# Wu0409/DuPL

Measured on AMD Instinct MI355X. Metric: training img/s at 448^2, VOC dual-student ViT-B/16, phase B step, higher is better.
Workload: dtype f32 storage / accumulation / results; Linear GEMMs (forward, dgrad, wgrad), attention (forward, backward) and the decoder convs as fp32-equivalent f16x3 split products on the f16 MFMA (operands as fp16 hi / lo planes, 3 products per block, fp32 accumulate; error vs fp64 <= the f32 MFMA kernels'); CA

## Files before the change

dupl_amd/csrc/gemm_split.hip:

```cpp
#include "split_frag.h"
#include "../../include/dupl_hip.h"

#ifndef G16_ABL
#define G16_ABL 0
#endif

namespace {

constexpr int TBK = 32;

template <bool F1>
__global__ __launch_bounds__(256) void split_kernel(const float* __restrict__ x, __half* __restrict__ hi, __half* __restrict__ lo,
                                                    long n4, float scale) {
    for (long i = (long)blockIdx.x * blockDim.x + threadIdx.x; i < n4; i += (long)gridDim.x * blockDim.x) {
        const float4 v = reinterpret_cast<const float4*>(x)[i];
        __half h[4], l[4];
        if constexpr (F1) {
            split_f32_u(v.x * scale, h[0], l[0]);
            split_f32_u(v.y * scale, h[1], l[1]);
            split_f32_u(v.z * scale, h[2], l[2]);
            split_f32_u(v.w * scale, h[3], l[3]);
        } else {
            split_f32(v.x, h[0], l[0]);
            split_f32(v.y, h[1], l[1]);
// ... 375 lines not shown
    const bool pre_ld = !ACC && E.vec && nv == 4 && ((p.res != nullptr) != want_aux);
    const float* pre_src = want_aux ? p.aux : p.res;
    const int pre_ldm = want_aux ? p.ldaux : p.ldr;
#pragma unroll
    for (int i = 0; i < WM; ++i)
#pragma unroll
        for (int g = 0; g < 4; ++g) {
            f32x4 pq[2] = {f32x4{0.f, 0.f, 0.f, 0.f}, f32x4{0.f, 0.f, 0.f, 0.f}};
            if (pre_ld) {
#pragma unroll
                for (int k = 0; k < 2; ++k) {
                    const int row = mw + i * 32 + 8 * g + rl + 4 * k;
                    if (row < p.M) pq[k] = *reinterpret_cast<const f32x4*>(pre_src + (size_t)row * pre_ldm + col);
                }
            }
#pragma unroll
            for (int j = 0; j < WN; ++j)
#pragma unroll
                for (int q = 0; q < 4; ++q)
                {
                    float v;
                    if constexpr (SINGLE) v = accM[i][j][4 * g + q] * alpha;
                    else v = (accM[i][j][4 * g + q] + accX[SINGLE ? 0 : i][SINGLE ? 0 : j][4 * g + q] * LO_INV) * alpha;
                    side[(q + 4 * hf) * 64 + j * 32 + l31] = v;
                }
            if constexpr (ACC) {
                if (OVERW && (p.flags & DUPL_GEMM_C_FRESH)) {
                    if (nw + lane < p.N) {
#pragma unroll
                        for (int r = 0; r < 8; ++r) {
                            const int row = mw + i * 32 + 8 * g + r;
                            if (row < p.M) p.C[(size_t)row * p.ldc + nw + lane] = 0.f + side[r * 64 + lane];
                        }
                    }
                } else if (nw + lane < p.N) {
#pragma unroll
                    for (int r = 0; r < 8; ++r) {
                        const int row = mw + i * 32 + 8 * g + r;
                        if (row < p.M) {
                            float* cp = p.C + (size_t)row * p.ldc + nw + lane;
                            if constexpr (ATOM) unsafeAtomicAdd(cp, side[r * 64 + lane]);
                            else *cp += side[r * 64 + lane];
                        }
                    }
                }
            } else {
#pragma unroll
                for (int k = 0; k < 2; ++k) {
                    const int r = rl + 4 * k;
                    const f32x4 t = *reinterpret_cast<const f32x4*>(side + r * 64 + cl);
                    const int row = mw + i * 32 + 8 * g + r;
                    if (nv > 0 && row < p.M)
                        epi16_quad(p, E, row, col, nv, t, bv, amx, pq[k], pre_ld ? (want_aux ? 2 : 1) : 0);
                }
            }
        }
}

template <int WM, int WN, int NWM, int NWN>
struct RingGeom {
    static constexpr int BM = 32 * WM * NWM, BN = 32 * WN * NWN, NW = NWM * NWN;
    static constexpr int PA = BM / 16, PB = BN / 16;
    static constexpr int NP = 2 * PA + 2 * PB;
    static constexpr int STAGE = NP * 1024;
    static constexpr int PPW = NP / NW;
    static constexpr int NMF = 3 * WM * WN, NR = 2 * (WM + WN);
    static_assert(NP % NW == 0, "pieces must divide over the waves");
};

template <int BM, int BN>
struct TileOrder {
    int nbm, g_gm, nblk, q8, r8, gspan;
    __device__ __forceinline__ TileOrder(const int nbm_, const int nbn, const int g_gm_)
        : nbm(nbm_), g_gm(g_gm_), nblk(nbm_ * nbn), q8(nblk >> 3), r8(nblk & 7), gspan(g_gm_ * nbn) {}
    __device__ __forceinline__ void lid_origin(const int lid, int& m0, int& n0) const {
        const int gid = lid / gspan, gin = lid - gid * gspan;
        const int gfirst = gid * g_gm;
        const int gsz = min(nbm - gfirst, g_gm);
        m0 = (gfirst + gin % gsz) * BM;
        n0 = (gin / gsz) * BN;
    }
    __device__ __forceinline__ void tile_origin(const int bid, int& m0, int& n0) const {
        const int xcd = bid & 7, idx = bid >> 3;
        lid_origin((xcd < r8 ? xcd * (q8 + 1) : r8 * (q8 + 1) + (xcd - r8) * q8) + idx, m0, n0);
    }
    __device__ __forceinline__ bool has_tile(const int bid) const { return (bid >> 3) < q8 + ((bid & 7) < r8 ? 1 : 0); }
};

__device__ __forceinline__ void g16_dma_piece(const char*& gp, char* dst) {
    if (!(G16_ABL & 1))
        __builtin_amdgcn_global_load_lds((const __attribute__((address_space(1))) void*)gp, (__attribute__((address_space(3))) void*)dst,
                                         16, 0, 0);
    gp += TBK * 2;
}

template <int WM, int WN, int PA, int PB>
struct Frag32 {
    int a_row, b_row;
    __device__ __forceinline__ void read_frags(const char* st, const int cs, h8 (&fa)[2 * WM], h8 (&fb)[2 * WN]) const {
#pragma unroll
        for (int i = 0; i < WM; ++i) {
            fa[i] = *reinterpret_cast<const h8*>(st + a_row + i * 2048 + cs);
            fa[WM + i] = *reinterpret_cast<const h8*>(st + PA * 1024 + a_row + i * 2048 + cs);
        }
#pragma unroll
        for (int j = 0; j < WN; ++j) {
// ... 944 lines not shown
        for (; t < nt; ++t) {
            const int nb = rb + 1 == STAGES ? 0 : rb + 1;
            const char* st = smem + rb * STAGE;
            const unsigned so = (unsigned)(rb * STAGE), son = (unsigned)(nb * STAGE);
            __builtin_amdgcn_s_waitcnt(LGKM0);
            phase(std::integral_constant<int, NRI>{}, f0a, f0b, [&](auto sc) __attribute__((always_inline)) { read_r(sc, KS1, st, so, f1a, f1b); });
            if (t + 1 < nt) {
                __builtin_amdgcn_s_waitcnt(WAIT_LGKM0_VM(0));
                __builtin_amdgcn_s_barrier();
                asm volatile("" ::: "memory");
                phase(std::integral_constant<int, NRI>{}, f1a, f1b, [&](auto sc) __attribute__((always_inline)) { read_r(sc, KS0, smem + nb * STAGE, son, f0a, f0b); });
            } else {
                __builtin_amdgcn_s_waitcnt(LGKM0);
                phase(std::integral_constant<int, 0>{}, f1a, f1b, [](auto) {});
            }
            rb = nb;
        }
        asm volatile("s_waitcnt lgkmcnt(0)" ::: "memory");
        __builtin_amdgcn_s_barrier();
        asm volatile("" ::: "memory");
        const int mw = m0 + wm * (32 * WM), nw = n0 + wn * (32 * WN);
        bool more;
        if constexpr (SK) {
            pos += nt;
            more = pos < pend;
            if (more) {
                nt = min(pend - pos, ntf);
                order.lid_origin(pos / ntf, m0, n0);
                plan(m0, n0, 0);
            }
        } else if constexpr (ONESHOT) {
            more = false;
        } else {
            bid += grid;
            more = order.has_tile(bid);
            if (more) {
                order.tile_origin(bid, m0, n0);
                plan(m0, n0, 0);
            }
        }
        if (more) {
#pragma unroll
            for (int s = 0; s < STAGES; ++s) issue(s);
        }
        gemm16_epilogue_side<WM, WN, ACC != 0, true, ACC == 1, ONESHOT>(p, acc, accX_unused, reinterpret_cast<float*>(smem + STAGES * STAGE) + wave * 512,
                                                               mw, nw, lane, amx);
        if (!more) break;
    }
    if (p.amax_out)
        gemm16_amax_flush(static_cast<unsigned int*>(p.amax_out), amx, reinterpret_cast<float*>(smem + STAGES * STAGE), wave, lane,
                          NWM * NWN);
}

template <int WM, int WN, int NWM, int NWN, int WPS, bool SK, int ACC, bool AKM, bool BKM, int STAGES = 3>
__global__ __launch_bounds__(64 * NWM * NWN, WPS) void gemm_f16x3_km_kernel(const dupl_gemm16_desc p, const int g_gm) {
    gemm_f16x3_km_body<WM, WN, NWM, NWN, WPS, SK, ACC, AKM, BKM, STAGES>(p, g_gm, blockIdx.x, gridDim.x);
}

struct g16_group_args {
    dupl_gemm16_desc d[DUPL_GEMM16_GROUP_MAX];
    int first[DUPL_GEMM16_GROUP_MAX + 1];
    int n;
};
template <int WM, int WN, int NWM, int NWN, int WPS>
__global__ __launch_bounds__(64 * NWM * NWN, WPS) void gemm_f16x3_km_group_kernel(const g16_group_args g, const int g_gm) {
    const int T = g.first[g.n];
    const int xcd = blockIdx.x & 7, idx = blockIdx.x >> 3;
    const int lo = (int)((long)T * xcd / 8), hi = (int)((long)T * (xcd + 1) / 8);
    if (idx >= hi - lo) return;
    const int t = lo + idx;
    int i = 0;
#pragma unroll 1
    while (i + 1 < g.n && t >= g.first[i + 1]) ++i;
    i = __builtin_amdgcn_readfirstlane(i);
    gemm_f16x3_km_body<WM, WN, NWM, NWN, WPS, false, 2, true, true, 3, true>(g.d[i], g_gm, t - g.first[i], 1 << 28);
}

}

constexpr int G16_GROUP_M = 8;
constexpr int G16_GROUP_RING = 2;
constexpr int G16_F1_BIG_FROM = 96;

extern "C" int dupl_split_f16x2(const float* x, void* hi, void* lo, int64_t n, dupl_stream_t stream) {
    if (!x || !hi || !lo || n <= 0 || (n & 3) || (reinterpret_cast<uintptr_t>(x) & 15) || (reinterpret_cast<uintptr_t>(hi) & 7) ||
        (reinterpret_cast<uintptr_t>(lo) & 7))
        return DUPL_ERR_ARG;
    const long n4 = n / 4;
    long g = (n4 + 255) / 256;
    if (g > 8192) g = 8192;
    DUPL_LAUNCH(split_kernel<false>, dim3((unsigned)g), dim3(256), 0, (hipStream_t)stream, x, (__half*)hi, (__half*)lo, n4, 1.f);
    return dupl_launch_status();
}

extern "C" int dupl_split_f16x2b(const float* x, void* hi, void* lo, int64_t n, int32_t scale_exp, dupl_stream_t stream) {
    if (!x || !hi || !lo || n <= 0 || (n & 3) || (reinterpret_cast<uintptr_t>(x) & 15) || (reinterpret_cast<uintptr_t>(hi) & 7) ||
        (reinterpret_cast<uintptr_t>(lo) & 7) || scale_exp < 0 || scale_exp > 15)
        return DUPL_ERR_ARG;
    const long n4 = n / 4;
    long g = (n4 + 255) / 256;
    if (g > 8192) g = 8192;
    DUPL_LAUNCH(split_kernel<true>, dim3((unsigned)g), dim3(256), 0, (hipStream_t)stream, x, (__half*)hi, (__half*)lo, n4,
                       ldexpf(1.f, scale_exp));
    return dupl_launch_status();
}

static bool g16_operands_ok(const dupl_gemm16_desc& d) {
    if (d.struct_size != sizeof(dupl_gemm16_desc)) return false;
    if (!d.A_hi || !d.A_lo || !d.B_hi || !d.B_lo || d.M <= 0 || d.N <= 0 || d.K <= 0) return false;
    if ((d.K % TBK) || (d.lda % 8) || (d.ldb % 8)) return false;
    auto al16 = [](const void* q) { return (reinterpret_cast<uintptr_t>(q) & 15) == 0; };
    if (!al16(d.A_hi) || !al16(d.A_lo) || !al16(d.B_hi) || !al16(d.B_lo)) return false;
    if (d.group < 0 || d.group > 4096) return false;
    if (d.a_layout < 0 || d.a_layout > 1 || d.b_layout < 0 || d.b_layout > 1 || d.ka_valid < 0 || d.kb_valid < 0) return false;
    if (d.a_layout || d.b_layout) {
        if (d.fmt != 1 || d.K / TBK < 3) return false;
        if ((d.a_layout && (d.M & 7)) || (d.b_layout && (d.N & 7))) return false;
        if (d.ka_valid > d.K || d.kb_valid > d.K) return false;
        if ((!d.a_layout && d.ka_valid) || (!d.b_layout && d.kb_valid)) return false;
    }
    return true;
}

extern "C" int dupl_gemm_f16x3_group(const dupl_gemm16_desc* descs, int32_t n, dupl_stream_t stream) {
    if (!descs || n < 1 || n > DUPL_GEMM16_GROUP_MAX) return DUPL_ERR_ARG;
    g16_group_args g;
    g.n = n;
    int total = 0, group = 0;
    for (int i = 0; i < n; ++i) {
        const dupl_gemm16_desc& d = descs[i];
        if (!g16_operands_ok(d)) return DUPL_ERR_ARG;
        if ((d.flags & ~DUPL_GEMM_C_FRESH) != DUPL_GEMM_ACCUM || d.a_layout != 1 || d.b_layout != 1) return DUPL_ERR_ARG;
        if (!d.C || d.C_hi || d.C_lo || d.bias || d.res || d.c_rows || d.amax_out) return DUPL_ERR_ARG;
        g.d[i] = d;
        g.first[i] = total;
        const int nblk = ((d.M + 255) / 256) * ((d.N + 127) / 128);
        total += nblk;
        if (d.group) group = d.group;
    }
    g.first[n] = total;
    DUPL_LAUNCH((gemm_f16x3_km_group_kernel<2, 2, 4, 2, 2>), dim3((unsigned)(8 * ((total + 7) / 8))), dim3(512), 0, (hipStream_t)stream, g,
                       group ? group : G16_GROUP_RING);
    return dupl_launch_status();
}

static bool g16_split_rows(const dupl_gemm16_desc& d, const int M1, dupl_gemm16_desc& d1, dupl_gemm16_desc& d2) {
    d1 = d; d2 = d;
    d1.M = M1;
    d2.M = d.M - M1;
    auto adv = [&](const void* q, size_t elems, size_t bytes) { return q ? static_cast<const void*>(static_cast<const char*>(q) + elems * bytes) : nullptr; };
    d2.A_hi = adv(d.A_hi, (size_t)M1 * d.lda, 2); d2.A_lo = adv(d.A_lo, (size_t)M1 * d.lda, 2);
    d2.C = (float*)adv(d.C, (size_t)M1 * d.ldc, 4);
    d2.C_hi = (void*)adv(d.C_hi, (size_t)M1 * d.ldo, 2); d2.C_lo = (void*)adv(d.C_lo, (size_t)M1 * d.ldo, 2);
    d2.res = (const float*)adv(d.res, (size_t)M1 * d.ldr, 4);
    d2.aux = (float*)adv(d.aux, (size_t)M1 * d.ldaux, 4);
    if (d.c_rows > 0) {
        if (d.c_rows <= M1) {
            d2.c_rows = 0; d2.C = nullptr; d2.aux = nullptr; d2.flags &= ~DUPL_GEMM_STORE_PRE;
        } else { d1.c_rows = 0; d2.c_rows = d.c_rows - M1; }
    }
    return d2.C || d2.C_hi;
}

constexpr int G16_TILES[] = {
    0,
    3,
    5,
    6,
    7,
    8,
    10,
    11,
    12,
    14,
    18,
    22,
};

static int g16_tile16(const dupl_gemm16_desc& d) {
    return ((d.M + 255) / 256) * ((d.N + 255) / 256) >= G16_F1_BIG_FROM ? 18 : 22;
}
using g16_kernel_t = void (*)(dupl_gemm16_desc, int);
static void g16_launch16(const dupl_gemm16_desc& d, const int t, const bool automatic, const int group, hipStream_t s, g16_kernel_t big,
                         g16_kernel_t small) {
    auto launch = [&](g16_kernel_t k, const dupl_gemm16_desc& q, const int bn) {
        DUPL_LAUNCH(k, dim3((unsigned)(((q.M + 255) / 256) * ((q.N + bn - 1) / bn))), dim3(512), 0, s, q, group);
    };
    if (t == 22) return launch(small, d, 128);
    const int cn = (d.N + 255) / 256, rm = (d.M + 255) / 256, cus = 256;
    const int nb22 = rm * cn, full = nb22 / cus, tail = nb22 - full * cus;
    const int r_big = full > 0 ? (full * cus) / cn : 0;
    dupl_gemm16_desc d1, d2;
    if (automatic && full > 0 && tail > 0 && tail * 10 < cus * 3 && r_big > 0 && r_big < rm && !d.amax_out && g16_split_rows(d, r_big * 256, d1, d2)) {
        launch(big, d1, 256);
        launch(small, d2, 128);
    } else launch(big, d, 256);
}

static int g16_launch_hi(const dupl_gemm16_desc& d, const int tile, const int group, hipStream_t s);

extern "C" int dupl_gemm_f16x3(const dupl_gemm16_desc* d, dupl_stream_t stream) {
    if (!d) return DUPL_ERR_ARG;
    dupl_gemm16_desc hi1;
    const bool single = d->struct_size == sizeof(dupl_gemm16_desc) && d->products == 1;
    if (single) {
        hi1 = *d;
        if (!hi1.A_lo) hi1.A_lo = hi1.A_hi;
        if (!hi1.B_lo) hi1.B_lo = hi1.B_hi;
        d = &hi1;
    }
    if (!g16_operands_ok(*d)) return DUPL_ERR_ARG;
    if (d->products != 0 && d->products != 1 && d->products != 3) return DUPL_ERR_ARG;
    if (d->concurrency < 0 || d->concurrency > 8 || d->persist_blocks < 0 || d->persist_blocks > 1024 || (d->persist_blocks & 7))
        return DUPL_ERR_ARG;
    bool known_tile = false;
    for (const int t : G16_TILES) known_tile |= d->tile == t;
    if (!known_tile) return DUPL_ERR_ARG;
    const int g16_tile = d->tile, g16_concurrency = d->concurrency > 0 ? d->concurrency : 1;
    const int g16_persist_blocks = d->persist_blocks ? d->persist_blocks : (g16_concurrency >= 2 ? 192 : 256);
    const int g16_group_m = d->group ? d->group : G16_GROUP_M, g16_group_ring = d->group ? d->group : G16_GROUP_RING;
    if (!d->C && !d->C_hi) return DUPL_ERR_ARG;
    if ((d->C_hi == nullptr) != (d->C_lo == nullptr)) return DUPL_ERR_ARG;
    if ((d->flags & (DUPL_GEMM_STORE_PRE | DUPL_GEMM_MUL_DGELU | DUPL_GEMM_MUL_RELUMASK)) && !d->aux) return DUPL_ERR_ARG;
    if (d->flags & ~(DUPL_GEMM_GELU | DUPL_GEMM_RELU | DUPL_GEMM_STORE_PRE | DUPL_GEMM_ACCUM | DUPL_GEMM_MUL_DGELU |
                     DUPL_GEMM_MUL_RELUMASK))
        return DUPL_ERR_ARG;
    const bool accum = d->flags & DUPL_GEMM_ACCUM;
    if (accum && (!d->C || d->C_hi || d->bias || d->res || d->c_rows)) return DUPL_ERR_ARG;
    if (d->c_rows < 0 || (d->c_rows && (d->flags & (DUPL_GEMM_MUL_DGELU | DUPL_GEMM_MUL_RELUMASK)))) return DUPL_ERR_ARG;
    if (d->amax_out && (accum || d->c_rows || (reinterpret_cast<uintptr_t>(d->amax_out) & 3))) return DUPL_ERR_ARG;
    const bool kmajor = d->a_layout || d->b_layout;
    if (d->fmt < 0 || d->fmt > 1 || d->out_exp < 0 || d->out_exp > 15 || (d->out_exp && d->fmt != 1) ||
        (d->fmt == 1 && !kmajor && (accum || d->amax_out)))
        return DUPL_ERR_ARG;
    hipStream_t s = (hipStream_t)stream;
    if (single) {
        if (accum || kmajor) return DUPL_ERR_ARG;
        return g16_launch_hi(*d, g16_tile, g16_group_ring, s);
    }
    int ksplit = 1;
    if (accum) {
        const long tiles = (long)((d->M + 127) / 128) * ((d->N + 127) / 128);
        ksplit = (int)((512 + tiles - 1) / tiles);
        const int maxs = (d->K / TBK + 7) / 8;
        if (ksplit > maxs) ksplit = maxs;
        if (ksplit < 1) ksplit = 1;
        if (d->deterministic) ksplit = 1;
    }
    int tile = g16_tile;
    if (tile == 0) {
        const long b256 = (long)((d->M + 255) / 256) * ((d->N + 127) / 128);
        const long b128 = (long)((d->M + 127) / 128) * ((d->N + 127) / 128) * ksplit;
        const bool ring = b256 >= (g16_concurrency >= 2 ? 64 : 128);
        if (!accum && ring) tile = 10;
        else if (accum && ksplit > 1 && d->K / TBK >= 8 && b256 * (d->K / TBK) >= 10L * g16_persist_blocks &&
                 (g16_concurrency < 2 || b256 >= 64))
            tile = 11;
        else tile = b128 < 200 ? 3 : 5;
    }
    auto blocks = [&](int bm, int bn) { return dim3((unsigned)(((d->M + bm - 1) / bm) * ((d->N + bn - 1) / bn)), (unsigned)ksplit); };
    auto persist_grid = [&](const int nblk) {
        const int tx = (nblk + 7) / 8, bmax = g16_persist_blocks / 8;
        const int rounds = (tx + bmax - 1) / bmax;
        return dim3((unsigned)(8 * ((tx + rounds - 1) / rounds)));
    };
    if (kmajor) {
        const int nb21 = ((d->M + 255) / 256) * ((d->N + 127) / 128);
        const bool sk = accum && !d->deterministic && ksplit > 1;
        dupl_gemm16_desc dsk = *d;
        if (accum) {
            const int ntf = d->K / TBK;
            auto per = [&](int s_) { return (ntf + s_ - 1) / s_; };
            auto fits = [&](int s_) { return s_ > 0 && (long)nb21 * s_ <= g16_persist_blocks && per(s_) >= 3 && ntf - (s_ - 1) * per(s_) >= 3; };
            if (dsk.sk_slices > 0 && !fits(dsk.sk_slices)) dsk.sk_slices = 0;
            if (dsk.sk_slices == 0) {
                int S = nb21 > g16_persist_blocks ? -1 : g16_persist_blocks / nb21;
                while (S > 1 && (per(S) < 3 || ntf - (S - 1) * per(S) < 3)) --S;
                dsk.sk_slices = S;
            }
            if (dsk.sk_slices > 0 && !fits(dsk.sk_slices)) dsk.sk_slices = -1;
        }
        if (accum && !d->a_layout) {
            if (!d->b_layout || d->deterministic) return DUPL_ERR_ARG;
            DUPL_LAUNCH((gemm_f16x3_km_kernel<2, 2, 4, 2, 2, true, 1, false, true>), dim3((unsigned)g16_persist_blocks), dim3(512), 0, s, dsk, g16_group_ring);
        } else if (accum) {
            if (!(d->a_layout && d->b_layout)) return DUPL_ERR_ARG;
            if (sk) DUPL_LAUNCH((gemm_f16x3_km_kernel<2, 2, 4, 2, 2, true, 1, true, true>), dim3((unsigned)g16_persist_blocks), dim3(512), 0, s, dsk, g16_group_ring);
            else DUPL_LAUNCH((gemm_f16x3_km_kernel<2, 2, 4, 2, 2, false, 2, true, true>), persist_grid(nb21), dim3(512), 0, s, *d, g16_group_ring);
        } else {
            if (d->a_layout || !d->b_layout) return DUPL_ERR_ARG;
            DUPL_LAUNCH((gemm_f16x3_km_kernel<2, 2, 4, 2, 2, false, 0, false, true>), persist_grid(nb21), dim3(512), 0, s, *d, g16_group_ring);
        }
        return dupl_launch_status();
    }
    if (d->fmt == 1) {
        const int nb21 = ((d->M + 255) / 256) * ((d->N + 127) / 128);
        int t = (g16_tile == 8 || g16_tile == 12 || g16_tile == 14 || g16_tile == 18 || g16_tile == 22) ? g16_tile : g16_tile16(*d);
        if (d->K / TBK < 3 && t == 14) t = 12;
        if (t == 18 || t == 22)
            g16_launch16(*d, t, g16_tile == 0, g16_group_ring, s, gemm_f16x3_ring16_kernel<4, 2, 2, 4, 2, 2>, gemm_f16x3_ring16_kernel<2, 2, 4, 2, 2, 3>);
        else if (t == 8) DUPL_LAUNCH((gemm_f16x3_ring_kernel<4, 2, 2, 4, 2, 2, true>), blocks(256, 256), dim3(512), 0, s, *d, g16_group_ring);
        else if (t == 12) DUPL_LAUNCH((gemm_f16x3_ring_kernel<2, 2, 4, 2, 2, 3, true>), blocks(256, 128), dim3(512), 0, s, *d, g16_group_ring);
        else
            DUPL_LAUNCH((gemm_f16x3_pring_kernel<2, 2, 4, 2, 2, false, true, 3>), persist_grid(nb21), dim3(512), 0, s, *d, g16_group_ring);
        return dupl_launch_status();
    }
    if (tile == 10 && (accum || d->K / TBK < 3)) tile = 6;
    if (tile == 11 && (!accum || d->deterministic || d->K / TBK < 8)) tile = accum ? 5 : 6;
    if (tile == 11) {
        DUPL_LAUNCH((gemm_f16x3_pring_kernel<2, 2, 4, 2, 2, true>), dim3((unsigned)g16_persist_blocks), dim3(512), 0, s, *d,
                           g16_group_ring);
        return dupl_launch_status();
    }
    if (tile == 10) {
        DUPL_LAUNCH((gemm_f16x3_pring_kernel<2, 2, 4, 2, 2>), persist_grid(((d->M + 255) / 256) * ((d->N + 127) / 128)), dim3(512), 0, s, *d,
                    g16_group_ring);
        return dupl_launch_status();
    }
    if (tile == 8 || tile == 12 || tile == 14 || tile == 18 || tile == 22) tile = 5;
    if (tile == 6) DUPL_LAUNCH((gemm_f16x3_ring_kernel<2, 2, 4, 2, 2>), blocks(256, 128), dim3(512), 0, s, *d, g16_group_ring);
    else if (tile == 7) DUPL_LAUNCH((gemm_f16x3_ring_kernel<4, 2, 2, 2, 1>), blocks(256, 128), dim3(256), 0, s, *d, g16_group_ring);
    else if (tile == 3) DUPL_LAUNCH((gemm_f16x3_kernel<2, 1, 2, 2, 2>), blocks(128, 64), dim3(256), 0, s, *d, g16_group_m);
    else DUPL_LAUNCH((gemm_f16x3_kernel<2, 1, 2, 4, 4>), blocks(128, 128), dim3(512), 0, s, *d, g16_group_m);
    return dupl_launch_status();
}

#ifndef G16H_STAGES
#define G16H_STAGES 4
#endif
static int g16_launch_hi(const dupl_gemm16_desc& d, const int tile, const int group, hipStream_t s) {
    const g16_kernel_t small = gemm_f16x3_ring16_kernel<2, 2, 4, 2, 2, G16H_STAGES, 1>, big = gemm_f16x3_ring16_kernel<4, 2, 2, 4, 2, G16H_STAGES, 1>;
    g16_launch16(d, (tile == 18 || tile == 22) ? tile : g16_tile16(d), tile == 0, group, s, big, small);
    return dupl_launch_status();
}
```

dupl_amd/ops.py:

```python
from __future__ import annotations

import ctypes
import os
from typing import Optional, Sequence

import numpy as np
import torch

from . import _lib
from ._lib import GemmDesc

Tensor = torch.Tensor


def L():
    return _lib.lib()


_DETERMINISTIC = [os.environ.get("DUPL_DETERMINISTIC", "0") == "1"]


def deterministic() -> bool:
    return _DETERMINISTIC[0]

# ... 275 lines not shown
    d.A_hi, d.A_lo, d.B_hi, d.B_lo = x.hi, x.lo, W.hi, W.lo
    d.C = _p(y)
    d.C_hi, d.C_lo = (y16.hi, y16.lo) if y16 is not None else (None, None)
    d.bias, d.res, d.aux = _p(bias), _p(res), _p(store_pre)
    d.M, d.N, d.K = M, N, K
    d.lda, d.ldb = x.cols, W.cols
    d.ldc = y.stride(0) if y is not None else 0
    d.ldo = N
    d.ldr = res.stride(0) if res is not None else 0
    d.ldaux = store_pre.stride(0) if store_pre is not None else 0
    aux_flag = _lib.GEMM_MUL_DGELU if dgelu_of is not None else (_lib.GEMM_MUL_RELUMASK if relumask_of is not None else
                                                                  (_lib.GEMM_STORE_PRE if store_pre is not None else 0))
    d.flags = (_lib.GEMM_GELU if gelu else 0) | (_lib.GEMM_RELU if relu else 0) | aux_flag | (_lib.GEMM_ACCUM if accumulate else 0)
    if isinstance(alpha, _Alpha):
        alpha.check()
    d.alpha_dev = int(alpha) if alpha is not None else None
    d.c_rows = int(c_rows)
    tn = tuning if tuning is not None else GEMM16_TUNING
    d.tile, d.concurrency = tn["tile"], tn["concurrency"]
    d.persist_blocks, d.group = tn["persist_blocks"], tn["group"]
    d.sk_slices = tn["sk_slices"]
    d.products = int(products)
    tok = None
    if amax_for_next and y is not None and not accumulate and not c_rows:
        d.amax_out, tok = reserve_amax(dev)
    if c_rows:
        assert y16 is not None and (y is None or y.shape[0] >= c_rows) and (store_pre is None or store_pre.shape[0] >= c_rows)
    L().dupl_gemm_f16x3(ctypes.byref(d), _stream())
    if tok is not None:
        y._dupl_amax = tok
    return y, y16


def wgrad16_group(items, tuning: Optional[dict] = None, fresh=None):
    descs = []
    assert fresh is None or len(fresh) == len(items)
    for j, (dy16, x16, out, alpha) in enumerate(items):
        assert dy16.fmt == 1 and getattr(x16, "fmt", 0) == 1, "grouped weight gradients read format 1 planes k-major"
        Kp = dy16.rows
        assert Kp % 32 == 0 and Kp >= 96 and out.is_contiguous() and out.shape == (dy16.cols, x16.cols)
        if isinstance(alpha, _Alpha):
            alpha.check()
        d = _lib.Gemm16Desc()
        d.deterministic = int(deterministic())
        d.A_hi, d.A_lo, d.B_hi, d.B_lo = dy16.hi, dy16.lo, x16.hi, x16.lo
        d.C = out.data_ptr()
        d.M, d.N, d.K = dy16.cols, x16.cols, Kp
        d.lda, d.ldb, d.ldc, d.ldo = dy16.cols, x16.cols, out.stride(0), x16.cols
        d.flags = _lib.GEMM_ACCUM | (_lib.GEMM_C_FRESH if fresh is not None and fresh[j] else 0)
        d.alpha_dev = int(alpha) if alpha is not None else None
        d.fmt, d.post_scale = 1, 2.0 ** -(getattr(dy16, "exp", 0) + getattr(x16, "exp", 0))
        d.a_layout, d.b_layout = 1, 1
        d.ka_valid, d.kb_valid = Kp, min(x16.rows, Kp)
        d.group = (tuning if tuning is not None else GEMM16_TUNING)["group"]
        descs.append(d)
    for i in range(0, len(descs), _lib.GEMM16_GROUP_MAX):
        chunk = descs[i:i + _lib.GEMM16_GROUP_MAX]
        arr = (_lib.Gemm16Desc * len(chunk))(*chunk)
        L().dupl_gemm_f16x3_group(arr, len(chunk), _stream())


def linear(x: Tensor, W: Tensor, bias: Optional[Tensor] = None, *, gelu: bool = False, relu: bool = False,
           res: Optional[Tensor] = None, out: Optional[Tensor] = None, store_pre: Optional[Tensor] = None) -> Tensor:
    M, K = x.shape
    N = W.shape[0]
    assert W.numel() == N * K
    y = out if out is not None else torch.empty((M, N), device=x.device, dtype=torch.float32)
    fl = (_lib.GEMM_GELU if gelu else 0) | (_lib.GEMM_RELU if relu else 0)
    if store_pre is not None:
        fl |= _lib.GEMM_STORE_PRE
    gemm_raw(x.data_ptr(), W.data_ptr(), y.data_ptr(), M, N, K, x.stride(0), K, y.stride(0), flags=fl,
             bias=_p(bias), res=_p(res), ldr=(res.stride(0) if res is not None else 0),
             aux=_p(store_pre), ldaux=(store_pre.stride(0) if store_pre is not None else 0))
    return y


def linear_dgrad(dy: Tensor, W: Tensor, *, dgelu_of: Optional[Tensor] = None, relumask_of: Optional[Tensor] = None,
                 out: Optional[Tensor] = None, accumulate: bool = False) -> Tensor:
    M, N = dy.shape
    K = W.numel() // N
    dx = out if out is not None else torch.empty((M, K), device=dy.device, dtype=torch.float32)
    fl = _lib.GEMM_B_NCONTIG | (_lib.GEMM_ACCUM if accumulate else 0)
    aux = None
    if dgelu_of is not None:
        fl |= _lib.GEMM_MUL_DGELU
        aux = dgelu_of
    if relumask_of is not None:
        fl |= _lib.GEMM_MUL_RELUMASK
        aux = relumask_of
    gemm_raw(dy.data_ptr(), W.data_ptr(), dx.data_ptr(), M, K, N, dy.stride(0), K, dx.stride(0), flags=fl,
             aux=_p(aux), ldaux=(aux.stride(0) if aux is not None else 0))
    return dx


def linear_wgrad(dy: Tensor, x: Tensor, out: Tensor, accumulate: bool = False):
    M, N = dy.shape
    K = x.shape[1]
    assert out.numel() == N * K
    fl = _lib.GEMM_A_MCONTIG | _lib.GEMM_B_NCONTIG | (_lib.GEMM_ACCUM if accumulate else 0)
    gemm_raw(dy.data_ptr(), x.data_ptr(), out.data_ptr(), N, K, M, dy.stride(0), x.stride(0), K, flags=fl)


def colsum(x: Tensor, out: Tensor, accumulate: bool = False):
    M, N = x.shape
    L().dupl_colsum(x.data_ptr(), out.data_ptr(), M, N, x.stride(0), int(accumulate), int(deterministic()), _stream())


# ... 659 lines not shown
```

Baseline: 85.36.

## Add 16x16x32 MFMA variant of k-major f16x3 GEMM for dgrad and wgrad

Adds a new k-major split-f16 GEMM body built on the 16x16x32 f16 MFMA instead of the 32x32 shape. It comes with its own interleaved LDS read, DMA and MFMA schedule and a matching side-buffer epilogue. By default (automatic tile) it is used for dgrad with and without split-K, non-split-K wgrad, and grouped wgrad. The aim is better MFMA throughput and overlap of LDS reads with compute for the backward GEMMs. In exchange it adds a large new code path with a different accumulator layout and epilogue row mapping, which may carry correctness and register-pressure risk.

After: 86.28 (median of 6 runs). 1.01x the previous value.

```diff
diff --git a/dupl_amd/csrc/gemm_split.hip b/dupl_amd/csrc/gemm_split.hip
--- a/dupl_amd/csrc/gemm_split.hip
+++ b/dupl_amd/csrc/gemm_split.hip
@@ -451,6 +451,69 @@
                     const int row = mw + i * 32 + 8 * g + r;
                     if (nv > 0 && row < p.M)
                         epi16_quad(p, E, row, col, nv, t, bv, amx, pq[k], pre_ld ? (want_aux ? 2 : 1) : 0);
+                }
+            }
+        }
+}
+
+template <bool ACC, bool ATOM, bool OVERW>
+__device__ __forceinline__ void gemm16_epilogue_side16(const dupl_gemm16_desc& p, f32x4 (&acc)[4][4], float* __restrict__ side, const int mw,
+                                                       const int nw, const int lane, float& amx) {
+    const int l15 = lane & 15, g = lane >> 4;
+    const float alpha = (p.alpha_dev ? *p.alpha_dev : 1.f) * (p.post_scale != 0.f ? p.post_scale : 1.f);
+    const Epi16 E = epi16_setup(p);
+    const int cl = l15 * 4, rl = g;
+    const int col = nw + cl;
+    const int nv = min(4, p.N - col);
+    float bv[4] = {0.f, 0.f, 0.f, 0.f};
+    if (!ACC && p.bias && nv > 0) {
+#pragma unroll
+        for (int c = 0; c < 4; ++c)
+            if (c < nv) bv[c] = p.bias[col + c];
+    }
+    const bool want_aux = E.f_dgelu || E.f_rmask;
+    const bool pre_ld = !ACC && E.vec && nv == 4 && ((p.res != nullptr) != want_aux);
+    const float* pre_src = want_aux ? p.aux : p.res;
+    const int pre_ldm = want_aux ? p.ldaux : p.ldr;
+    auto tile_row = [](const int i, const int ep, const int s) { return 16 * i + 4 * (s >> 1) + 2 * ep + (s & 1); };
+#pragma unroll
+    for (int i = 0; i < 4; ++i)
+#pragma unroll
+        for (int ep = 0; ep < 2; ++ep) {
+            f32x4 pq[2] = {f32x4{0.f, 0.f, 0.f, 0.f}, f32x4{0.f, 0.f, 0.f, 0.f}};
+            if (pre_ld) {
+#pragma unroll
+                for (int k = 0; k < 2; ++k) {
+                    const int row = mw + tile_row(i, ep, rl + 4 * k);
+                    if (row < p.M) pq[k] = *reinterpret_cast<const f32x4*>(pre_src + (size_t)row * pre_ldm + col);
+                }
+            }
+#pragma unroll
+            for (int j = 0; j < 4; ++j)
+#pragma unroll
+                for (int de = 0; de < 2; ++de) side[(2 * g + de) * 64 + ((j * 16 + l15 + 16 * g) & 63)] = acc[i][j][2 * ep + de] * alpha;
+            if constexpr (ACC) {
+                if (nw + lane < p.N) {
+                    const bool fresh = OVERW && (p.flags & DUPL_GEMM_C_FRESH);
+#pragma unroll
+                    for (int r = 0; r < 8; ++r) {
+                        const int row = mw + tile_row(i, ep, r);
+                        if (row < p.M) {
+                            float* cp = p.C + (size_t)row * p.ldc + nw + lane;
+                            const float v = side[r * 64 + ((lane + 16 * (r >> 1)) & 63)];
+                            if (fresh) *cp = 0.f + v;
+                            else if constexpr (ATOM) unsafeAtomicAdd(cp, v);
+                            else *cp += v;
+                        }
+                    }
+                }
+            } else {
+#pragma unroll
+                for (int k = 0; k < 2; ++k) {
+                    const int s = rl + 4 * k;
+                    const f32x4 t = *reinterpret_cast<const f32x4*>(side + s * 64 + ((cl + 16 * (s >> 1)) & 63));
+                    const int row = mw + tile_row(i, ep, s);
+                    if (nv > 0 && row < p.M) epi16_quad(p, E, row, col, nv, t, bv, amx, pq[k], pre_ld ? (want_aux ? 2 : 1) : 0);
                 }
             }
         }
@@ -1501,9 +1564,305 @@
                           NWM * NWN);
 }
 
-template <int WM, int WN, int NWM, int NWN, int WPS, bool SK, int ACC, bool AKM, bool BKM, int STAGES = 3>
+template <int WM, int WN, int NWM, int NWN, int WPS, bool SK, int ACC, bool AKM, bool BKM, int STAGES = 3, bool ONESHOT = false>
+__device__ __forceinline__ void gemm_f16x3_km16_body(const dupl_gemm16_desc& p, const int g_gm, const int bid0, const int grid) {
+    using G = RingGeom<WM, WN, NWM, NWN>;
+    constexpr int BM = G::BM, BN = G::BN, NW = G::NW, PA = G::PA, PB = G::PB, STAGE = G::STAGE, PPW = G::PPW;
+    constexpr int APW = 2 * PA / NW;
+    constexpr int RB = 2 * WM, CB = 2 * WN;
+    constexpr int NDA = AKM ? 2 : 1, NDB = BKM ? 2 : 1;
+    constexpr int NLA = 4 * NDA, NLB = 2 * NDB;
+    constexpr int SIDE = NW * 2048;
+    static_assert(RB == 4 && CB == 4, "wave tile 64 x 64: two phases of two row blocks, the 4 x 4 side-buffer epilogue");
+    static_assert((2 * PA) % NW == 0, "pieces must divide over the waves, operand by operand");
+    static_assert(STAGES * STAGE + SIDE <= 160 * 1024, "LDS");
+    static_assert(!SK || ACC == 1, "stream-K pieces meet in atomics");
+    __shared__ __attribute__((aligned(1024))) char smem[STAGES * STAGE + SIDE];
+    const int tid = threadIdx.x;
+    const int lane = tid & 63, wave = __builtin_amdgcn_readfirstlane(tid >> 6);
+    const int wm = wave / NWN, wn = wave % NWN;
+    const int nbm = (p.M + BM - 1) / BM, nbn = (p.N + BN - 1) / BN;
+    const int ntf = p.K / TBK;
+    int nt = ntf;
+    const TileOrder<BM, BN> order(nbm, nbn, g_gm);
+
+    const int ka_valid = p.ka_valid > 0 ? p.ka_valid : p.K, kb_valid = p.kb_valid > 0 ? p.kb_valid : p.K;
+    const unsigned lda2 = __builtin_amdgcn_readfirstlane(p.lda * 2), ldb2 = __builtin_amdgcn_readfirstlane(p.ldb * 2);
+    const char* gp[PPW];
+    int prow[PPW];
+    int kt = 0;
+    auto plan = [&](const int m0, const int n0, const int k0) __attribute__((always_inline)) {
+#pragma unroll
+        for (int i = 0; i < PPW; ++i) {
+            const int g = wave + NW * i;
+            const bool isA = i < APW;
+            const int gg = isA ? g : g - 2 * PA;
+            const int PO = isA ? PA : PB;
+            const bool lo = gg >= PO;
+            const int q = lo ? gg - PO : gg;
+            const __half* plane = static_cast<const __half*>(isA ? (lo ? p.A_lo : p.A_hi) : (lo ? p.B_lo : p.B_hi));
+            const int ld = isA ? p.lda : p.ldb, r0 = isA ? m0 : n0, R = isA ? p.M : p.N;
+            const bool km = isA ? AKM : BKM;
+            if (!km) {
+                const int pr = lane >> 2;
+                const int jsrc = (lane & 3) ^ ((4 - (pr >> 2)) & 3);
+                const int row = min(r0 + q * 16 + pr, R - 1);
+                gp[i] = reinterpret_cast<const char*>(plane + (size_t)row * ld + (size_t)k0 * TBK) + jsrc * 16;
+                prow[i] = 0;
+            } else {
+                const int NPH = (isA ? BM : BN) / 32;
+                const int jj = q / NPH, dp = q - jj * NPH;
+                const int col = min(r0 + dp * 32 + km16_piece_col_bytes(0, lane) / 2, R - 8);
+                gp[i] = reinterpret_cast<const char*>(plane + col);
+                prow[i] = km16_piece_row(jj << 1, lane);
+            }
+        }
+        kt = k0;
+    };
+    auto dma_piece = [&](const int i, char* dst) __attribute__((always_inline)) {
+        const bool km = (i < APW) ? AKM : BKM;
+        if (!km) g16_dma_piece(gp[i], dst + i * (NW * 1024));
+        else {
+            const int kv = (i < APW) ? ka_valid : kb_valid;
+            const int krow = min(kt * TBK + prow[i], kv - 1);
+            __builtin_amdgcn_global_load_lds((const __attribute__((address_space(1))) void*)(gp[i] + (size_t)krow * ((i < APW) ? lda2 : ldb2)),
+                                             (__attribute__((address_space(3))) void*)(dst + i * (NW * 1024)), 16, 0, 0);
+        }
+    };
+    auto issue = [&](int buf) __attribute__((always_inline)) {
+        char* dst = smem + buf * STAGE + wave * 1024;
+#pragma unroll
+        for (int i = 0; i < PPW; ++i) dma_piece(i, dst);
+        ++kt;
+    };
+
+    const int l15 = lane & 15;
+    const int ch = ((lane >> 4) ^ ((4 - (l15 >> 2)) & 3)) * 16;
+    const int a_off = (wm * (32 * WM) + l15) * 64 + ch, b_off = 2 * PA * 1024 + (wn * (32 * WN) + l15) * 64 + ch;
+    const unsigned lds0 = (unsigned)(uintptr_t)((__attribute__((address_space(3))) char*)smem);
+    const unsigned akm0 = lds0 + km16_read_lane_off(lane) + wm * RB * 512, bkm0 = lds0 + 2 * PA * 1024 + km16_read_lane_off(lane) + wn * CB * 512;
+
+    f32x4 acc[RB][CB];
+    h4 fa0[8], fa1[8], fb[4 * CB];
+    auto tr_off = [](const unsigned addr, auto offc) __attribute__((always_inline)) { return km_tr_read<decltype(offc)::value>(addr); };
+    auto read_a = [&](auto ric, auto phc, const char* st, const unsigned so, h4(&fa)[8]) __attribute__((always_inline)) {
+        constexpr int RI = decltype(ric)::value, PH = decltype(phc)::value;
+        constexpr int f = RI / NDA, half = RI % NDA, pl = f >> 1, rbk = 2 * PH + (f & 1);
+        if constexpr (!AKM) {
+            const h8 v = *reinterpret_cast<const h8*>(st + pl * (PA * 1024) + a_off + rbk * 1024);
+            fa[2 * f] = __builtin_shufflevector(v, v, 0, 1, 2, 3);
+            fa[2 * f + 1] = __builtin_shufflevector(v, v, 4, 5, 6, 7);
+        } else {
+            fa[2 * f + half] = tr_off(akm0 + so, std::integral_constant<int, pl * (PA * 1024) + (half * (BM / 16) + rbk) * 512>{});
+        }
+    };
+    auto read_b = [&](auto ric, auto jc, const char* st, const unsigned so) __attribute__((always_inline)) {
+        constexpr int RI = decltype(ric)::value, J = decltype(jc)::value;
+        constexpr int pl = RI / NDB, half = RI % NDB, f = pl * CB + J;
+        if constexpr (!BKM) {
+            const h8 v = *reinterpret_cast<const h8*>(st + pl * (PB * 1024) + b_off + J * 1024);
+            fb[2 * f] = __builtin_shufflevector(v, v, 0, 1, 2, 3);
+            fb[2 * f + 1] = __builtin_shufflevector(v, v, 4, 5, 6, 7);
+        } else {
+            fb[2 * f + half] = tr_off(bkm0 + so, std::integral_constant<int, pl * (PB * 1024) + (half * (BN / 16) + J) * 512>{});
+        }
+    };
+    auto frag = [](const h4 lo, const h4 hi) __attribute__((always_inline)) { return __builtin_shufflevector(lo, hi, 0, 1, 2, 3, 4, 5, 6, 7); };
+    auto mfma_n = [&](auto phc, auto jc, auto nc, const h4(&fa)[8]) __attribute__((always_inline)) {
+        constexpr int PH = decltype(phc)::value, J = decltype(jc)::value, n = decltype(nc)::value, pass = n / 2, k = n % 2;
+        constexpr int af = pass == 2 ? 2 + k : k, bf = pass == 1 ? CB + J : J;
+        acc[2 * PH + k][J] = __builtin_amdgcn_mfma_f32_16x16x32_f16(frag(fa[2 * af], fa[2 * af + 1]), frag(fb[2 * bf], fb[2 * bf + 1]),
+                                                                    acc[2 * PH + k][J], 0, 0, 0);
+    };
+    constexpr int NMB = 6;
+    auto block = [&](auto phc, auto jc, auto nsc, const h4(&fa)[8], auto&& slot) __attribute__((always_inline)) {
+        constexpr int NS = decltype(nsc)::value;
+        if constexpr (NS == 0) {
+            static_for<NMB>([&](auto nc) __attribute__((always_inline)) { mfma_n(phc, jc, nc, fa); });
+        } else {
+            static_for<NS>([&](auto sc) __attribute__((always_inline)) {
+                constexpr int S = decltype(sc)::value, n0 = S * NMB / NS, n1 = (S + 1) * NMB / NS;
+                slot(sc);
+                static_for<n1 - n0>([&](auto kc) __attribute__((always_inline)) { mfma_n(phc, jc, std::integral_constant<int, n0 + decltype(kc)::value>{}, fa); });
+                __builtin_amdgcn_sched_barrier(0);
+            });
+        }
+    };
+    auto wait_a = [](h4(&f)[8]) __attribute__((always_inline)) {
+        asm volatile("s_waitcnt lgkmcnt(0)" : "+v"(f[0]), "+v"(f[1]), "+v"(f[2]), "+v"(f[3]), "+v"(f[4]), "+v"(f[5]), "+v"(f[6]), "+v"(f[7]) : : "memory");
+    };
+    auto pin4 = [](h4& a, h4& b, h4& c, h4& d) __attribute__((always_inline)) { asm volatile("" : "+v"(a), "+v"(b), "+v"(c), "+v"(d) : : "memory"); };
+    auto pin_b = [&](auto jc) __attribute__((always_inline)) {
+        constexpr int J = decltype(jc)::value;
+        pin4(fb[2 * J], fb[2 * J + 1], fb[2 * (CB + J)], fb[2 * (CB + J) + 1]);
+    };
+    constexpr std::integral_constant<int, 0> P0{};
+    constexpr std::integral_constant<int, 1> P1{};
+    constexpr std::integral_constant<int, CB - 1> JL{};
+    auto k_tile = [&](auto loadc, auto dmac, auto vmc, const int rb, const int nb) __attribute__((always_inline)) {
+        constexpr bool LOAD = decltype(loadc)::value, DMA = decltype(dmac)::value;
+        const char* st = smem + rb * STAGE;
+        const char* nx = smem + nb * STAGE;
+        const unsigned so = (unsigned)(rb * STAGE), son = (unsigned)(nb * STAGE);
+        wait_a(fa0);
+        static_for<CB - 1>([&](auto jc) __attribute__((always_inline)) { pin_b(jc); });
+        __builtin_amdgcn_sched_barrier(0);
+        constexpr int NL0 = NLB + NLA;
+        static_for<CB - 1>([&](auto jc) __attribute__((always_inline)) {
+            constexpr int J = decltype(jc)::value, L0 = J * NL0 / (CB - 1), L1 = (J + 1) * NL0 / (CB - 1);
+            block(P0, jc, std::integral_constant<int, L1 - L0>{}, fa0, [&](auto sc) __attribute__((always_inline)) {
+                constexpr int L = L0 + decltype(sc)::value;
+                if constexpr (L < NLB) read_b(std::integral_constant<int, L>{}, JL, st, so);
+                else read_a(std::integral_constant<int, L - NLB>{}, P1, st, so, fa1);
+            });
+        });
+        wait_a(fa1);
+        pin_b(JL);
+        __builtin_amdgcn_sched_barrier(0);
+        block(P0, JL, std::integral_constant<int, 0>{}, fa0, [](auto) {});
+        __builtin_amdgcn_sched_barrier(0);
+        if constexpr (LOAD) {
+            __builtin_amdgcn_s_waitcnt(WAIT_LGKM0_VM(decltype(vmc)::value));
+            __builtin_amdgcn_s_barrier();
+            asm volatile("" ::: "memory");
+        }
+        char* dst = smem + rb * STAGE + wave * 1024;
+        static_for<CB>([&](auto jc) __attribute__((always_inline)) {
+            constexpr int J = decltype(jc)::value;
+            constexpr int D0 = DMA ? J * PPW / CB : 0, D1 = DMA ? (J + 1) * PPW / CB : 0;
+            constexpr int NRD = LOAD ? (J == 0 ? NLA : NLB) : 0;
+            block(P1, jc, std::integral_constant<int, NRD + (D1 - D0)>{}, fa1, [&](auto sc) __attribute__((always_inline)) {
+                constexpr int S = decltype(sc)::value;
+                if constexpr (S < NRD) {
+                    if constexpr (J == 0) read_a(sc, P0, nx, son, fa0);
+                    else read_b(sc, std::integral_constant<int, J - 1>{}, nx, son);
+                } else {
+                    constexpr int I = D0 + S - NRD;
+                    dma_piece(I, dst);
+                    if constexpr (I == PPW - 1) ++kt;
+                }
+            });
+        });
+        __builtin_amdgcn_sched_barrier(0);
+    };
+
+    int bid = bid0;
+    int pos = 0, pend = 0;
+    int m0, n0;
+    if constexpr (SK) {
+        const int T = order.nblk * ntf, G = grid;
+        if (p.sk_slices > 0) {
+            const int S = p.sk_slices, nblk = order.nblk, U = nblk * S;
+            const int xcd = bid & 7, idx = bid >> 3;
+            const int ulo = (int)((long)U * xcd / 8), uhi = (int)((long)U * (xcd + 1) / 8);
+            if (idx >= uhi - ulo) return;
+            const int u = ulo + idx;
+            const int slice = u / nblk, lid = u - slice * nblk;
+            const int per = (ntf + S - 1) / S;
+            const int k0 = slice * per;
+            nt = min(per, ntf - k0);
+            pos = lid * ntf + k0;
+            pend = pos + nt;
+            order.lid_origin(lid, m0, n0);
+            plan(m0, n0, k0);
+        } else {
+            const int L = (bid & 7) * (G >> 3) + (bid >> 3);
+            auto cut = [&](const int l) {
+                int x = (int)((long)T * l / G);
+                const int r = x % ntf;
+                if (r && r < 3) x -= r;
+                else if (r > ntf - 3) x += ntf - r;
+                return x;
+            };
+            pos = cut(L);
+            pend = cut(L + 1);
+            if (pos >= pend) return;
+            const int lid = pos / ntf, k0 = pos - lid * ntf;
+            nt = min(pend - pos, ntf - k0);
+            order.lid_origin(lid, m0, n0);
+            plan(m0, n0, k0);
+        }
+    } else if constexpr (ONESHOT) {
+        if (bid >= order.nblk) return;
+        order.lid_origin(bid, m0, n0);
+        plan(m0, n0, 0);
+    } else {
+        if (!order.has_tile(bid)) return;
+        order.tile_origin(bid, m0, n0);
+        plan(m0, n0, 0);
+    }
+#pragma unroll
+    for (int s = 0; s < STAGES; ++s) issue(s);
+    bool first = true;
+    float amx = 0.f;
+    for (;;) {
+#pragma unroll
+        for (int i = 0; i < RB; ++i)
+#pragma unroll
+            for (int j = 0; j < CB; ++j) acc[i][j] = f32x4{0.f, 0.f, 0.f, 0.f};
+        if (first) asm volatile("s_waitcnt vmcnt(%0)" ::"n"((STAGES - 1) * PPW) : "memory");
+        else asm volatile("s_waitcnt vmcnt(0)" ::: "memory");
+        first = false;
+        __builtin_amdgcn_s_barrier();
+        asm volatile("" ::: "memory");
+        static_for<NLA>([&](auto rc) __attribute__((always_inline)) { read_a(rc, P0, smem, 0u, fa0); });
+        static_for<CB - 1>([&](auto jc) __attribute__((always_inline)) {
+            static_for<NLB>([&](auto rc) __attribute__((always_inline)) { read_b(rc, jc, smem, 0u); });
+        });
+        __builtin_amdgcn_sched_barrier(0);
+        int rb = 0;
+        int t = 0;
+        for (; t + STAGES < nt; ++t) {
+            const int nb = rb + 1 == STAGES ? 0 : rb + 1;
+            k_tile(std::true_type{}, std::true_type{}, std::integral_constant<int, (STAGES - 2) * PPW>{}, rb, nb);
+            rb = nb;
+        }
+        for (; t + 1 < nt; ++t) {
+            const int nb = rb + 1 == STAGES ? 0 : rb + 1;
+            k_tile(std::true_type{}, std::false_type{}, std::integral_constant<int, 0>{}, rb, nb);
+            rb = nb;
+        }
+        k_tile(std::false_type{}, std::false_type{}, std::integral_constant<int, 0>{}, rb, rb);
+        asm volatile("s_waitcnt lgkmcnt(0)" ::: "memory");
+        __builtin_amdgcn_s_barrier();
+        asm volatile("" ::: "memory");
+        const int mw = m0 + wm * (32 * WM), nw = n0 + wn * (32 * WN);
+        bool more;
+        if constexpr (SK) {
+            pos += nt;
+            more = pos < pend;
+            if (more) {
+                nt = min(pend - pos, ntf);
+                order.lid_origin(pos / ntf, m0, n0);
+                plan(m0, n0, 0);
+            }
+        } else if constexpr (ONESHOT) {
+            more = false;
+        } else {
+            bid += grid;
+            more = order.has_tile(bid);
+            if (more) {
+                order.tile_origin(bid, m0, n0);
+                plan(m0, n0, 0);
+            }
+        }
+        if (more) {
+#pragma unroll
+            for (int s = 0; s < STAGES; ++s) issue(s);
+        }
+        gemm16_epilogue_side16<ACC != 0, ACC == 1, ONESHOT>(p, acc, reinterpret_cast<float*>(smem + STAGES * STAGE) + wave * 512, mw, nw, lane, amx);
+        if (!more) break;
+    }
+    if (p.amax_out)
+        gemm16_amax_flush(static_cast<unsigned int*>(p.amax_out), amx, reinterpret_cast<float*>(smem + STAGES * STAGE), wave, lane,
+                          NWM * NWN);
+}
+
+template <int WM, int WN, int NWM, int NWN, int WPS, bool SK, int ACC, bool AKM, bool BKM, int STAGES = 3, int MF = 32>
 __global__ __launch_bounds__(64 * NWM * NWN, WPS) void gemm_f16x3_km_kernel(const dupl_gemm16_desc p, const int g_gm) {
-    gemm_f16x3_km_body<WM, WN, NWM, NWN, WPS, SK, ACC, AKM, BKM, STAGES>(p, g_gm, blockIdx.x, gridDim.x);
+    static_assert(MF == 16 || MF == 32, "MFMA shape");
+    if constexpr (MF == 16) gemm_f16x3_km16_body<WM, WN, NWM, NWN, WPS, SK, ACC, AKM, BKM, STAGES>(p, g_gm, blockIdx.x, gridDim.x);
+    else gemm_f16x3_km_body<WM, WN, NWM, NWN, WPS, SK, ACC, AKM, BKM, STAGES>(p, g_gm, blockIdx.x, gridDim.x);
 }
 
 struct g16_group_args {
@@ -1511,7 +1870,7 @@
     int first[DUPL_GEMM16_GROUP_MAX + 1];
     int n;
 };
-template <int WM, int WN, int NWM, int NWN, int WPS>
+template <int WM, int WN, int NWM, int NWN, int WPS, int MF = 32>
 __global__ __launch_bounds__(64 * NWM * NWN, WPS) void gemm_f16x3_km_group_kernel(const g16_group_args g, const int g_gm) {
     const int T = g.first[g.n];
     const int xcd = blockIdx.x & 7, idx = blockIdx.x >> 3;
@@ -1522,7 +1881,8 @@
 #pragma unroll 1
     while (i + 1 < g.n && t >= g.first[i + 1]) ++i;
     i = __builtin_amdgcn_readfirstlane(i);
-    gemm_f16x3_km_body<WM, WN, NWM, NWN, WPS, false, 2, true, true, 3, true>(g.d[i], g_gm, t - g.first[i], 1 << 28);
+    if constexpr (MF == 16) gemm_f16x3_km16_body<WM, WN, NWM, NWN, WPS, false, 2, true, true, 3, true>(g.d[i], g_gm, t - g.first[i], 1 << 28);
+    else gemm_f16x3_km_body<WM, WN, NWM, NWN, WPS, false, 2, true, true, 3, true>(g.d[i], g_gm, t - g.first[i], 1 << 28);
 }
 
 }
@@ -1530,6 +1890,12 @@
 constexpr int G16_GROUP_M = 8;
 constexpr int G16_GROUP_RING = 2;
 constexpr int G16_F1_BIG_FROM = 96;
+
+constexpr bool KM16_DGRAD_EPI = true;
+constexpr bool KM16_DGRAD_SK = true;
+constexpr bool KM16_WGRAD_SK = false;
+constexpr bool KM16_WGRAD_TILE = true;
+static bool g16_km16(const int tile, const bool automatic) { return tile == 26 || (tile != 24 && automatic); }
 
 extern "C" int dupl_split_f16x2(const float* x, void* hi, void* lo, int64_t n, dupl_stream_t stream) {
     if (!x || !hi || !lo || n <= 0 || (n & 3) || (reinterpret_cast<uintptr_t>(x) & 15) || (reinterpret_cast<uintptr_t>(hi) & 7) ||
@@ -1575,7 +1941,7 @@
     if (!descs || n < 1 || n > DUPL_GEMM16_GROUP_MAX) return DUPL_ERR_ARG;
     g16_group_args g;
     g.n = n;
-    int total = 0, group = 0;
+    int total = 0, group = 0, tile = 0;
     for (int i = 0; i < n; ++i) {
         const dupl_gemm16_desc& d = descs[i];
         if (!g16_operands_ok(d)) return DUPL_ERR_ARG;
@@ -1586,10 +1952,14 @@
         const int nblk = ((d.M + 255) / 256) * ((d.N + 127) / 128);
         total += nblk;
         if (d.group) group = d.group;
+        if (d.tile) tile = d.tile;
     }
     g.first[n] = total;
-    DUPL_LAUNCH((gemm_f16x3_km_group_kernel<2, 2, 4, 2, 2>), dim3((unsigned)(8 * ((total + 7) / 8))), dim3(512), 0, (hipStream_t)stream, g,
-                       group ? group : G16_GROUP_RING);
+    const dim3 grid((unsigned)(8 * ((total + 7) / 8)));
+    if (g16_km16(tile, KM16_WGRAD_TILE))
+        DUPL_LAUNCH((gemm_f16x3_km_group_kernel<2, 2, 4, 2, 2, 16>), grid, dim3(512), 0, (hipStream_t)stream, g, group ? group : G16_GROUP_RING);
+    else
+        DUPL_LAUNCH((gemm_f16x3_km_group_kernel<2, 2, 4, 2, 2, 32>), grid, dim3(512), 0, (hipStream_t)stream, g, group ? group : G16_GROUP_RING);
     return dupl_launch_status();
 }
 
@@ -1624,6 +1994,8 @@
     14,
     18,
     22,
+    24,
+    26,
 };
 
 static int g16_tile16(const dupl_gemm16_desc& d) {
@@ -1665,7 +2037,9 @@
     bool known_tile = false;
     for (const int t : G16_TILES) known_tile |= d->tile == t;
     if (!known_tile) return DUPL_ERR_ARG;
-    const int g16_tile = d->tile, g16_concurrency = d->concurrency > 0 ? d->concurrency : 1;
+    const bool kmajor = d->a_layout || d->b_layout;
+    const int g16_tile = (d->tile == 24 || d->tile == 26) && !kmajor ? 0 : d->tile;
+    const int g16_concurrency = d->concurrency > 0 ? d->concurrency : 1;
     const int g16_persist_blocks = d->persist_blocks ? d->persist_blocks : (g16_concurrency >= 2 ? 192 : 256);
     const int g16_group_m = d->group ? d->group : G16_GROUP_M, g16_group_ring = d->group ? d->group : G16_GROUP_RING;
     if (!d->C && !d->C_hi) return DUPL_ERR_ARG;
@@ -1678,7 +2052,6 @@
     if (accum && (!d->C || d->C_hi || d->bias || d->res || d->c_rows)) return DUPL_ERR_ARG;
     if (d->c_rows < 0 || (d->c_rows && (d->flags & (DUPL_GEMM_MUL_DGELU | DUPL_GEMM_MUL_RELUMASK)))) return DUPL_ERR_ARG;
     if (d->amax_out && (accum || d->c_rows || (reinterpret_cast<uintptr_t>(d->amax_out) & 3))) return DUPL_ERR_ARG;
-    const bool kmajor = d->a_layout || d->b_layout;
     if (d->fmt < 0 || d->fmt > 1 || d->out_exp < 0 || d->out_exp > 15 || (d->out_exp && d->fmt != 1) ||
         (d->fmt == 1 && !kmajor && (accum || d->amax_out)))
         return DUPL_ERR_ARG;
@@ -1731,14 +2104,27 @@
         }
         if (accum && !d->a_layout) {
             if (!d->b_layout || d->deterministic) return DUPL_ERR_ARG;
-            DUPL_LAUNCH((gemm_f16x3_km_kernel<2, 2, 4, 2, 2, true, 1, false, true>), dim3((unsigned)g16_persist_blocks), dim3(512), 0, s, dsk, g16_group_ring);
+            if (g16_km16(g16_tile, KM16_DGRAD_SK))
+                DUPL_LAUNCH((gemm_f16x3_km_kernel<2, 2, 4, 2, 2, true, 1, false, true, 3, 16>), dim3((unsigned)g16_persist_blocks), dim3(512), 0, s, dsk, g16_group_ring);
+            else
+                DUPL_LAUNCH((gemm_f16x3_km_kernel<2, 2, 4, 2, 2, true, 1, false, true, 3, 32>), dim3((unsigned)g16_persist_blocks), dim3(512), 0, s, dsk, g16_group_ring);
         } else if (accum) {
             if (!(d->a_layout && d->b_layout)) return DUPL_ERR_ARG;
-            if (sk) DUPL_LAUNCH((gemm_f16x3_km_kernel<2, 2, 4, 2, 2, true, 1, true, true>), dim3((unsigned)g16_persist_blocks), dim3(512), 0, s, dsk, g16_group_ring);
-            else DUPL_LAUNCH((gemm_f16x3_km_kernel<2, 2, 4, 2, 2, false, 2, true, true>), persist_grid(nb21), dim3(512), 0, s, *d, g16_group_ring);
+            if (sk) {
+                if (g16_km16(g16_tile, KM16_WGRAD_SK))
+                    DUPL_LAUNCH((gemm_f16x3_km_kernel<2, 2, 4, 2, 2, true, 1, true, true, 3, 16>), dim3((unsigned)g16_persist_blocks), dim3(512), 0, s, dsk, g16_group_ring);
+                else
+                    DUPL_LAUNCH((gemm_f16x3_km_kernel<2, 2, 4, 2, 2, true, 1, true, true, 3, 32>), dim3((unsigned)g16_persist_blocks), dim3(512), 0, s, dsk, g16_group_ring);
+            } else if (g16_km16(g16_tile, KM16_WGRAD_TILE))
+                DUPL_LAUNCH((gemm_f16x3_km_kernel<2, 2, 4, 2, 2, false, 2, true, true, 3, 16>), persist_grid(nb21), dim3(512), 0, s, *d, g16_group_ring);
+            else
+                DUPL_LAUNCH((gemm_f16x3_km_kernel<2, 2, 4, 2, 2, false, 2, true, true, 3, 32>), persist_grid(nb21), dim3(512), 0, s, *d, g16_group_ring);
         } else {
             if (d->a_layout || !d->b_layout) return DUPL_ERR_ARG;
-            DUPL_LAUNCH((gemm_f16x3_km_kernel<2, 2, 4, 2, 2, false, 0, false, true>), persist_grid(nb21), dim3(512), 0, s, *d, g16_group_ring);
+            if (g16_km16(g16_tile, KM16_DGRAD_EPI))
+                DUPL_LAUNCH((gemm_f16x3_km_kernel<2, 2, 4, 2, 2, false, 0, false, true, 3, 16>), persist_grid(nb21), dim3(512), 0, s, *d, g16_group_ring);
+            else
+                DUPL_LAUNCH((gemm_f16x3_km_kernel<2, 2, 4, 2, 2, false, 0, false, true, 3, 32>), persist_grid(nb21), dim3(512), 0, s, *d, g16_group_ring);
         }
         return dupl_launch_status();
     }
diff --git a/dupl_amd/ops.py b/dupl_amd/ops.py
--- a/dupl_amd/ops.py
+++ b/dupl_amd/ops.py
@@ -351,7 +351,8 @@
         d.fmt, d.post_scale = 1, 2.0 ** -(getattr(dy16, "exp", 0) + getattr(x16, "exp", 0))
         d.a_layout, d.b_layout = 1, 1
         d.ka_valid, d.kb_valid = Kp, min(x16.rows, Kp)
-        d.group = (tuning if tuning is not None else GEMM16_TUNING)["group"]
+        tn = tuning if tuning is not None else GEMM16_TUNING
+        d.group, d.tile = tn["group"], tn["tile"]
         descs.append(d)
     for i in range(0, len(descs), _lib.GEMM16_GROUP_MAX):
         chunk = descs[i:i + _lib.GEMM16_GROUP_MAX]
```
